# ZwwWayne/mmMOT

Measured on AMD Instinct MI355X. Metric: frame-pairs/sec (fusion+affinity fwd) at N_det=64; affinity L∞ vs CPU ref, higher is better.
Workload: dtype f16x3

## Files before the change

### include/mmmot_hip.h

```cpp
#ifndef MMMOT_HIP_H
#define MMMOT_HIP_H

#include <stddef.h>
#include <stdint.h>

#ifdef __cplusplus
extern "C" {
#endif

#define MMMOT_OK 0
#define MMMOT_EINVAL (-1)

#define MMMOT_ACT_NONE 0
#define MMMOT_ACT_RELU 1
#define MMMOT_ACT_SIGMOID 2

#define MMMOT_A_PLAIN 0
#define MMMOT_A_NORM_RELU 1
#define MMMOT_A_PAIR 2

#define MMMOT_PAIR_MULTIPLY 0
#define MMMOT_PAIR_MINUS_ABS 1
#define MMMOT_PAIR_MINUS 2

// ... 49 lines not shown
int mmmot_conv3x3_raw_hl16(const void* in, const void* wp, const float* bias, float* out, int L, int H, int W, int Cin,
                           int Cout, const float* oscale, void* stream);

typedef struct mmmot_gemm_args {
  const float* X; int ldx;
  const float* W;
  const float* bias;
  const float* dbias; const int* rowidx; int lddb;
  float* Y; int ldy;
  float* part;
  const float* sc; const float* sh; int ldsc;
  const float* FA; const float* FB; int ldf;
  const int* tile_row0; const int* tile_nrows; const int* tile_group;
  const int* grp_row0; const int* grp_M; const int* grp_aoff; const int* grp_boff;
  int T; int N; int K;
  int amode; int pairop; int act;
  int w_hl16; float oscale;
  const float* osc; const float* osh; int ldosc;
  float* colsum;
  int pair_uniform32;
} mmmot_gemm_args;
int mmmot_gemm_rows(const mmmot_gemm_args* a, void* stream);
int mmmot_set_gemm_rows_variant(int v);

typedef struct mmmot_gemm_ares_args {
  const float* X; int ldx;
  const float* sc; const float* sh; int ldsc;
  const void* W;
  const float* bias;
  const float* dbias; const int* tile_dbrow; int lddb;
  const int* tile_row0; const int* tile_nrows; const int* tile_group;
  float* part;
  const float* osc; const float* osh; int ldosc;
  float* colsum;
  int T; int N; int K;
  float oscale;
} mmmot_gemm_ares_args;
int mmmot_gemm_ares(const mmmot_gemm_ares_args* a, void* stream);
int mmmot_set_gemm_ares_variant(int v);

int mmmot_gram_rows(const float* X, int ldx, int K, const float* sc, const float* sh, int ldsc,
                    const int* tile_row0, const int* tile_nrows, const int* tile_group, int T,
                    double* Gout, double* Sout, void* stream);
int mmmot_set_gram128_variant(int v);
int mmmot_gn_finalize_gram(const double* Gp, const double* Sp, const int* grp_tile0, const int* grp_ntiles,
                           const int* grp_count, int G, int K, const float* W, const float* bias, int N,
// ... 9 lines not shown
                      const float* gamma, const float* beta, float eps,
                      float* sc, float* sh, void* stream);

int mmmot_segment_mean(const float* X, int ldx, int C,
                       const int* seg_start, const int* seg_count, const int* seg_stride,
                       const int* seg_group, const int* seg_div, int nseg,
                       const float* sc, const float* sh, int ldsc, int relu,
                       float* out, int ldo,
                       int hl16 ,
                       void* stream);

int mmmot_rowdot(const float* X, int ldx, int K, const float* w, float b,
                 const float* sc, const float* sh, int ldsc,
                 const int* tile_row0, const int* tile_nrows, const int* tile_group, int T,
                 int act, int use_thr, float thr,
                 float* out, const int* omap, void* stream);

int mmmot_row_layernorm(const float* X, int ldx, int C, const float* gamma, const float* beta,
                        float eps, int relu, float* Y, int ldy, int R, void* stream);

int mmmot_skippool_head(const float* P, int ldp, int C, int C4, const float* g0, const float* b0, const float* w1,
                        const float* c1, const float* g2, const float* b2, const float* w4, const float* c4,
                        const float* g5, const float* b5, float eps, float* out, int ldo, int R, void* stream);
int mmmot_pointnet_layer1(const float* X, int K, const float* W, const float* bias,
                          float* Y, float* part,
                          const int* tile_row0, const int* tile_nrows, int T, void* stream);

int mmmot_pn_mlp64(const float* X, int ldx, const float* sc, const float* sh, int ldsc, const void* W16,
                   float oscale, const float* bias, float* Y, int ldy, float* part, const int* tile_row0,
                   const int* tile_nrows, const int* tile_group, int T, int N, void* stream);

int mmmot_affine_act(const float* X, int ldx, int C, const float* sc, const float* sh, int ldsc,
                     const int* tile_row0, const int* tile_nrows, const int* tile_group, int T,
                     int act, float* Y, int ldy, void* stream);

int mmmot_fusion_combine(int mode, const float* cat, const float* Y0, int ld0,
                         const float* Y1, int ld1,
                         const float* sc0, const float* sh0, const float* sc1, const float* sh1, int ldsc,
                         const int* tile_row0, const int* tile_nrows, const int* tile_group, int T,
                         float* F, int Lt, int C, void* stream);

int mmmot_softmax_pairs(const float* logits, float* out,
                        const int* grp_row0, const int* grp_N, const int* grp_M, int G,
                        int max_nm ,
                        int mode, void* stream);

// ... 103 lines not shown
```

### mmmot_amd/_lib.py

```python
import ctypes
import os
import subprocess
import threading

_HERE = os.path.dirname(os.path.abspath(__file__))
CSRC = os.path.join(_HERE, 'csrc')
LIB_PATH = os.environ.get('MMMOT_LIB_PATH', os.path.join(_HERE, 'libmmmot_hip.so'))
SOURCES = ['conv3x3.hip', 'hl16_format.hip', 'conv3x3_hl16_patch.hip', 'gemm_rows.hip', 'gemm_wide.hip',
           'gemm_ares.hip', 'gemm_wres.hip', 'gemm_wreg.hip', 'pn_mlp64.hip', 'gram.hip', 'points_gather.hip', 'crop_resize.hip', 'small_kernels.hip', 'backward.hip', 'train.hip', 'train_vgg.hip', 'gemm_tn_f16.hip',
           'assign.hip', 'track_ids.hip']
HIPCC = os.environ.get('HIPCC', '/opt/rocm/bin/hipcc')
HIPFLAGS = ['--offload-arch=gfx950', '-O3', '-std=c++17', '-fPIC']

_lock = threading.Lock()
_lib = None

c_f = ctypes.c_void_p
c_i = ctypes.c_int


class GemmArgs(ctypes.Structure):
    _fields_ = [
        ('X', c_f), ('ldx', c_i),
        ('W', c_f),
# ... 23 lines not shown
        ('dbias', c_f), ('tile_dbrow', c_f), ('lddb', c_i),
        ('tile_row0', c_f), ('tile_nrows', c_f), ('tile_group', c_f),
        ('part', c_f),
        ('osc', c_f), ('osh', c_f), ('ldosc', c_i),
        ('colsum', c_f),
        ('T', c_i), ('N', c_i), ('K', c_i),
        ('oscale', ctypes.c_float),
    ]


class GemmTnArgs(ctypes.Structure):
    _fields_ = [
        ('dY', c_f), ('lddy', c_i),
        ('X', c_f), ('ldx', c_i),
        ('sc', c_f), ('sh', c_f), ('ldsc', c_i),
        ('FA', c_f), ('FB', c_f), ('ldf', c_i),
        ('tile_row0', c_f), ('tile_nrows', c_f), ('tile_group', c_f),
        ('grp_row0', c_f), ('grp_M', c_f), ('grp_aoff', c_f), ('grp_boff', c_f),
        ('T', c_i), ('N', c_i), ('K', c_i), ('amode', c_i), ('pairop', c_i), ('nsplit', c_i),
        ('dW', c_f), ('db', c_f),
    ]


SIGNATURES = {
    'mmmot_abi_version': [],
    'mmmot_device_info': [c_i, ctypes.POINTER(c_i), ctypes.c_char_p, c_i],
    'mmmot_conv3x3_bn_relu': [c_f, c_f, c_f, c_f, c_i, c_i, c_i, c_i, c_i, c_i, c_i, c_f],
    'mmmot_gemm_rows': [ctypes.POINTER(GemmArgs), c_f],
    'mmmot_set_gemm_rows_variant': [c_i],
    'mmmot_gemm_ares': [ctypes.POINTER(GemmAresArgs), c_f],
    'mmmot_set_gemm_ares_variant': [c_i],
    'mmmot_gram_rows': [c_f, c_i, c_i, c_f, c_f, c_i, c_f, c_f, c_f, c_i, c_f, c_f, c_f],
    'mmmot_set_gram128_variant': [c_i],
    'mmmot_gn_finalize_gram': [c_f, c_f, c_f, c_f, c_f, c_i, c_i, c_f, c_f, c_i, c_f, c_f, ctypes.c_float, c_f, c_f, c_f, c_f],
    'mmmot_gn_finalize_gram_dbias': [c_f, c_f, c_f, c_f, c_f, c_i, c_f, c_f, c_i, c_f, c_f, c_i, c_i, c_f, c_f, ctypes.c_float,
                                     c_f, c_f, c_f, c_f],
    'mmmot_gn_finalize': [c_f, c_f, c_f, c_f, c_f, c_i, c_i, c_i, c_i, c_f, c_f, ctypes.c_float, c_f, c_f, c_f],
    'mmmot_segment_mean': [c_f, c_i, c_i, c_f, c_f, c_f, c_f, c_f, c_i, c_f, c_f, c_i, c_i, c_f, c_i, c_i, c_f],
    'mmmot_conv3x3_bn_relu_hl16_patch': [c_f, c_f, c_f, c_f, c_i, c_i, c_i, c_i, c_i, c_i, c_f, c_f],
    'mmmot_conv1_fused_hl16': [c_f, c_f, c_f, ctypes.c_float, c_f, c_f, c_f, c_f, c_i, c_i, c_i, c_f],
    'mmmot_conv3x3_bn_relu_hq8': [c_f, c_f, c_f, c_f, c_i, c_i, c_i, c_i, c_i, c_i, c_f, c_f],
    'mmmot_conv1_fused_u8': [c_f, ctypes.c_float, ctypes.c_float, ctypes.c_float, ctypes.c_float, ctypes.c_float,
                             ctypes.c_float, c_f, c_f, ctypes.c_float, c_f, c_f, c_f, c_f, c_i, c_i, c_i, c_i, c_f],
    'mmmot_u8_normalize': [c_f, c_i, c_i, c_f, c_f, c_f],
    'mmmot_conv1_fused_hq8': [c_f, c_f, c_f, ctypes.c_float, c_f, c_f, c_f, c_f, c_i, c_i, c_i, c_f],
    'mmmot_conv3x3_first_hl16': [c_f, c_f, c_f, c_f, c_i, c_i, c_i, c_i, c_f],
    'mmmot_set_patch_grid_limit': [c_i],
    'mmmot_set_patch_min_block': [c_i],
    'mmmot_trunk_range_read': [ctypes.POINTER(ctypes.c_uint), c_i],
    'mmmot_trunk_range_bind': [c_f],
    'mmmot_hl16_pack': [c_f, c_f, ctypes.c_long, c_f],
    'mmmot_hl16_unpack': [c_f, c_f, ctypes.c_long, c_f],
    'mmmot_hl16_pack_pow2': [c_f, c_f, ctypes.c_long, c_f, c_i, c_f],
    'mmmot_pow2_oscale': [c_f, c_i, c_f, c_i, c_f, c_i, c_f],
    'mmmot_conv3x3_raw_hl16': [c_f, c_f, c_f, c_f, c_i, c_i, c_i, c_i, c_i, c_f, c_f],
    'mmmot_hq8_pack': [c_f, c_f, ctypes.c_long, c_f],
    'mmmot_hq8_unpack': [c_f, c_f, ctypes.c_long, c_f],
    'mmmot_rowdot': [c_f, c_i, c_i, c_f, ctypes.c_float, c_f, c_f, c_i, c_f, c_f, c_f, c_i, c_i, c_i,
                     ctypes.c_float, c_f, c_f, c_f],
    'mmmot_row_layernorm': [c_f, c_i, c_i, c_f, c_f, ctypes.c_float, c_i, c_f, c_i, c_i, c_f],
    'mmmot_skippool_head': [c_f, c_i, c_i, c_i, c_f, c_f, c_f, c_f, c_f, c_f, c_f, c_f, c_f, c_f, ctypes.c_float, c_f, c_i, c_i,
                            c_f],
    'mmmot_pointnet_layer1': [c_f, c_i, c_f, c_f, c_f, c_f, c_f, c_f, c_i, c_f],
    'mmmot_pn_mlp64': [c_f, c_i, c_f, c_f, c_i, c_f, ctypes.c_float, c_f, c_f, c_i, c_f, c_f, c_f, c_f, c_i, c_i, c_f],
    'mmmot_affine_act': [c_f, c_i, c_i, c_f, c_f, c_i, c_f, c_f, c_f, c_i, c_i, c_f, c_i, c_f],
    'mmmot_fusion_combine': [c_i, c_f, c_f, c_i, c_f, c_i, c_f, c_f, c_f, c_f, c_i, c_f, c_f, c_f, c_i, c_f,
                             c_i, c_i, c_f],
    'mmmot_softmax_pairs': [c_f, c_f, c_f, c_f, c_f, c_i, c_i, c_i, c_f],
    'mmmot_points_count': [c_f, c_i, c_i, c_f, c_i, c_i, c_f, c_f, c_f],
    'mmmot_points_scatter': [c_f, c_i, c_i, c_f, c_i, c_f, c_f, c_f, c_i, c_f],
    'mmmot_crop_resize_norm': [c_f, c_i, c_i, c_f, c_i, c_i, c_i, c_f, c_f, c_f, c_f, c_f],
    'mmmot_points_count_batched': [c_f, c_i, c_i, c_i, c_i, c_i, c_f, c_f, c_f, c_f, c_f, c_f, c_f, c_i, c_f, c_f, c_f],
    'mmmot_points_scatter_batched': [c_f, c_i, c_i, c_i, c_i, c_i, c_f, c_f, c_f, c_f, c_f, c_f, c_f, c_f, c_f, c_f, c_i, c_f],
    'mmmot_selftest_mfma': [c_f, c_f, c_f, c_i, c_f],
    'mmmot_gn_bwd_partial': [c_f, c_i, c_f, c_i, c_i, c_f, c_f, c_i, c_f, c_f, c_i, c_f, c_f, c_f, c_i, c_f, c_f],
    'mmmot_gn_bwd_finalize': [c_f, c_f, c_i, c_i, c_i, c_f, c_f, c_f],
    'mmmot_gn_bwd_apply': [c_f, c_i, c_f, c_i, c_i, c_f, c_f, c_i, c_f, c_f, c_i, c_f, c_f, c_f, c_f, c_i, c_f, c_i, c_f],
    'mmmot_gemm_tn': [ctypes.POINTER(GemmTnArgs), c_f],
    'mmmot_gemm_tn_f16': [ctypes.POINTER(GemmTnArgs), c_f, c_f],
    'mmmot_absmax': [c_f, c_i, ctypes.c_long, c_i, c_f, c_f],
    'mmmot_pair_bwd': [c_f, c_i, c_f, c_i, c_f, c_i, c_i, c_f, c_f, c_f, c_f, c_f, c_f, c_f, c_i, c_i, c_i, c_f],
    'mmmot_pair_expand_bwd': [c_f, c_i, c_f, c_i, c_i, c_f, c_f, c_f, c_i, c_f, c_f, c_f, c_f, c_f],
    'mmmot_rowdot_bwd': [c_f, c_i, c_i, c_f, ctypes.c_float, c_f, c_f, c_i, c_f, c_f, c_f, c_i, c_i, c_f, c_f, c_f, c_i,
                         c_f, c_i, c_f],
    'mmmot_softmax_pairs_bwd': [c_f, c_f, c_f, c_f, c_f, c_f, c_i, c_i, c_i, c_f],
# ... 86 lines not shown
```

### mmmot_amd/csrc/gemm_rows.hip

```cpp
#include "common.h"

#define G16_BK 64
#define G16_LDT 72

template <int BN, int AMODE, bool F16>
__global__ __launch_bounds__(MM_THREADS, 2) void gemm_rows_kernel(mmmot_gemm_args a, int ntn) {
  constexpr int WM = (BN == 128) ? 2 : 4;
  constexpr int WN = 4 / WM;
  constexpr int TM = MM_BM / (WM * 32);
  constexpr int TN = BN / (WN * 32);
  constexpr int BLD = BN / 32;
  constexpr int BK = F16 ? G16_BK : MM_BK;
  constexpr int KV = BK / 32;
  constexpr int SMEM_BYTES = F16 ? (MM_BM + BN) * G16_LDT * 2 * 2 : (MM_BM + BN) * MM_LDT * 4;
  constexpr bool STAGED_OUT = F16 && BN == 128;

  __shared__ __attribute__((aligned(16))) unsigned char smem_raw[SMEM_BYTES];
  float* smem = reinterpret_cast<float*>(smem_raw);
  float* As = smem;
  float* Bs = smem + MM_BM * MM_LDT;
  _Float16* hs = reinterpret_cast<_Float16*>(smem_raw);
  _Float16* As_hi = hs;
  _Float16* As_lo = hs + MM_BM * G16_LDT;
  _Float16* Bs_hi = hs + 2 * MM_BM * G16_LDT;
// ... 289 lines not shown
                acc[tm][tn][e];
      __syncthreads();
      constexpr int C4 = BN / 4;
      for (int w = tid; w < MM_BM * C4; w += MM_THREADS) {
        const int r = w / C4, c = (w - r * C4) * 4;
        if (r < nrows) {
          f32x4 v = *reinterpret_cast<const f32x4*>(&Cs[r * CLD + c]);
#pragma unroll
          for (int e = 0; e < 4; ++e) v[e] = mm_act(v[e], a.act);
          *reinterpret_cast<f32x4*>(&a.Y[(long)(row0 + r) * a.ldy + n0 + c]) = v;
        }
      }
    }
  }
}

template <int BN, int AMODE, bool F16>
static int launch_gemm(const mmmot_gemm_args* a, hipStream_t s) {
  const int ntn = a->N / BN;
  hipLaunchKernelGGL((gemm_rows_kernel<BN, AMODE, F16>), dim3(a->T * ntn), dim3(MM_THREADS), 0, s, *a, ntn);
  return mm_check(hipGetLastError());
}

template <bool F16>
static int dispatch_gemm(const mmmot_gemm_args* a, hipStream_t s) {
  const bool wide = (a->N % 128 == 0);
  switch (a->amode) {
    case MMMOT_A_PLAIN:
      return wide ? launch_gemm<128, MMMOT_A_PLAIN, F16>(a, s) : launch_gemm<64, MMMOT_A_PLAIN, F16>(a, s);
    case MMMOT_A_NORM_RELU:
      return wide ? launch_gemm<128, MMMOT_A_NORM_RELU, F16>(a, s) : launch_gemm<64, MMMOT_A_NORM_RELU, F16>(a, s);
    case MMMOT_A_PAIR:
      return wide ? launch_gemm<128, MMMOT_A_PAIR, F16>(a, s) : launch_gemm<64, MMMOT_A_PAIR, F16>(a, s);
  }
  return MMMOT_EINVAL;
}

int mmmot_gemm_wide_try(const mmmot_gemm_args* a, hipStream_t s, int* status);

extern "C" int mmmot_gemm_rows(const mmmot_gemm_args* a, void* stream) {
  hipStream_t s = (hipStream_t)stream;
  if (!a || !a->W || a->T <= 0 || !a->tile_row0 || !a->tile_nrows) return MMMOT_EINVAL;
  const int bk = a->w_hl16 ? G16_BK : MM_BK;
  if (a->K <= 0 || a->K % bk != 0 || a->N <= 0 || a->N % 64 != 0) return MMMOT_EINVAL;
  if (!mm_al16(a->W)) return MMMOT_EINVAL;
  if (a->amode == MMMOT_A_PAIR) {
    if (!a->FA || !a->FB || !a->grp_row0 || !a->grp_M || !a->grp_aoff || !a->grp_boff || !a->tile_group)
      return MMMOT_EINVAL;
    if (a->ldf % 4 != 0 || !mm_al16(a->FA) || !mm_al16(a->FB)) return MMMOT_EINVAL;
  } else {
    if (!a->X || a->ldx % 4 != 0 || !mm_al16(a->X)) return MMMOT_EINVAL;
    if (a->amode == MMMOT_A_NORM_RELU &&
        (!a->sc || !a->sh || a->ldsc % 4 != 0 || !mm_al16(a->sc) || !mm_al16(a->sh)))
      return MMMOT_EINVAL;
  }
  if (a->dbias && !a->rowidx) return MMMOT_EINVAL;
  if (a->colsum && (!a->osc || !a->osh)) return MMMOT_EINVAL;
// ... 32 lines not shown
```

### mmmot_amd/csrc/small_kernels.hip

```cpp
#include "common.h"

__global__ __launch_bounds__(256) void gn_finalize_kernel(
    const float* __restrict__ part, const int* __restrict__ grp_tile0, const int* __restrict__ grp_ntiles,
    const int* __restrict__ grp_count, const int* __restrict__ tile_nrows, int ldp, int C, int NG,
    const float* __restrict__ gamma, const float* __restrict__ beta, float eps, float* __restrict__ sc,
    float* __restrict__ sh) {
  __shared__ double red[2][4];
  const int g = blockIdx.x / NG, ng = blockIdx.x % NG;
  const int CG = C / NG, c0 = ng * CG;
  const int tile0 = grp_tile0[g], nt = grp_ntiles[g];
  const int tid = threadIdx.x, lane = tid & 63, wave = tid >> 6;
  const int rows = grp_count[g];
  const int dq = 256 / CG, dr = 256 % CG;
  const int ti0 = tid / CG, cc0 = tid % CG;
  constexpr int U = 16;
  double s1 = 0.0;
  {
    int ti = ti0, cc = cc0;
    while (ti < nt) {
      float v[U];
      int n = 0;
#pragma unroll
      for (int u = 0; u < U; ++u) {
        v[u] = 0.f;
// ... 467 lines not shown
        const bool up = (lane & o) != 0;
#pragma unroll
        for (int i = 0; i < o; ++i) {
          const float keep = up ? acc[i + o] : acc[i];
          const float send = up ? acc[i] : acc[i + o];
          acc[i] = keep + __shfl_xor(send, o);
        }
      }
      const int jb = lane / ROWS, rr = lane % ROWS;
      if (j0 + jb < N) out[rr][j0 + jb] = acc[0] + bias[j0 + jb];
    } else {
#pragma unroll
      for (int jb = 0; jb < JB; ++jb)
#pragma unroll
        for (int rr = 0; rr < ROWS; ++rr) {
          const float t = wave_sum(acc[jb * ROWS + rr]);
          if (lane == 0 && j0 + jb < N) out[rr][j0 + jb] = t + bias[j0 + jb];
        }
    }
  }
}

template <int ROWS>
__global__ __launch_bounds__(256) void skippool_head_kernel(
    const float* __restrict__ P, int ldp, int C, int C4, const float* __restrict__ g0, const float* __restrict__ b0,
    const float* __restrict__ w1, const float* __restrict__ c1, const float* __restrict__ g2,
    const float* __restrict__ b2, const float* __restrict__ w4, const float* __restrict__ c4,
    const float* __restrict__ g5, const float* __restrict__ b5, float eps, float* __restrict__ out, int ldo, int R) {
  constexpr int JB = ROWS == 8 ? 8 : SP_JB;
  constexpr int RW = ROWS < 4 ? 1 : ROWS / 4;
  __shared__ __attribute__((aligned(16))) float xs[ROWS][512];
  __shared__ __attribute__((aligned(16))) float hs[ROWS][512];
  __shared__ float h1[ROWS][128];
  const int lane = threadIdx.x & 63, wave = threadIdx.x >> 6;
  const int row0 = blockIdx.x * ROWS;
#pragma unroll
  for (int q = 0; q < RW; ++q) {
    const int lr = wave * RW + q;
    if (lr < ROWS) sp_layernorm_row(P + (long)(row0 + lr < R ? row0 + lr : 0) * ldp, C, g0, b0, eps, false, xs[lr], lane);
  }
  __syncthreads();
  sp_matvec<ROWS, JB>(w1, c1, C4, C, xs, h1, lane, wave);
  __syncthreads();
#pragma unroll
  for (int q = 0; q < RW; ++q) {
    const int lr = wave * RW + q;
    if (lr < ROWS) sp_layernorm_row(h1[lr], C4, g2, b2, eps, true, hs[lr], lane);
  }
  __syncthreads();
  sp_matvec<ROWS, JB>(w4, c4, 128, C4, hs, h1, lane, wave);
  __syncthreads();
#pragma unroll
  for (int q = 0; q < RW; ++q) {
    const int lr = wave * RW + q;
    if (lr < ROWS && row0 + lr < R) sp_layernorm_row(h1[lr], 128, g5, b5, eps, true, out + (long)(row0 + lr) * ldo, lane);
  }
}

extern "C" int mmmot_skippool_head(const float* P, int ldp, int C, int C4, const float* g0, const float* b0,
                                   const float* w1, const float* c1, const float* g2, const float* b2, const float* w4,
                                   const float* c4, const float* g5, const float* b5, float eps, float* out, int ldo,
                                   int R, void* stream) {
  if (!P || !g0 || !b0 || !w1 || !c1 || !g2 || !b2 || !w4 || !c4 || !g5 || !b5 || !out || R <= 0) return MMMOT_EINVAL;
  if (C <= 0 || C % 64 != 0 || C > 512 || C4 <= 0 || C4 % 64 != 0 || C4 > 128) return MMMOT_EINVAL;
  if (!mm_al16(w1) || !mm_al16(w4)) return MMMOT_EINVAL;
  if (R >= 256)
    hipLaunchKernelGGL(skippool_head_kernel<8>, dim3((R + 7) / 8), dim3(256), 0, (hipStream_t)stream, P, ldp,
                       C, C4, g0, b0, w1, c1, g2, b2, w4, c4, g5, b5, eps, out, ldo, R);
  else
    hipLaunchKernelGGL(skippool_head_kernel<SP_ROWS>, dim3((R + SP_ROWS - 1) / SP_ROWS), dim3(256), 0, (hipStream_t)stream,
                       P, ldp, C, C4, g0, b0, w1, c1, g2, b2, w4, c4, g5, b5, eps, out, ldo, R);
  return mm_check(hipGetLastError());
}

template <int K>
__global__ __launch_bounds__(256) void pointnet_layer1_kernel(
    const float* __restrict__ X, const float* __restrict__ W, const float* __restrict__ bias,
    float* __restrict__ Y, float* __restrict__ part, const int* __restrict__ tile_row0,
    const int* __restrict__ tile_nrows) {
  __shared__ float xs[MM_BM * K];
  __shared__ float red[4][2][64];
  const int t = blockIdx.x;
  const int row0 = tile_row0[t], nrows = tile_nrows[t];
  const int tid = threadIdx.x;
  for (int idx = tid; idx < nrows * K; idx += 256) xs[idx] = X[(long)row0 * K + idx];
  __syncthreads();
  const int c = tid & 63, rq = tid >> 6;
  float w[K];
#pragma unroll
  for (int k = 0; k < K; ++k) w[k] = W[c * K + k];
  const float bv = bias[c];
  auto val = [&](int r) {
    float y = bv;
#pragma unroll
// ... 212 lines not shown
```

### mmmot_amd/engine.py

```python
import contextlib
import itertools
import os
import threading

import numpy as np
import torch

from .ops import (ACT_NONE, ACT_RELU, ACT_SIGMOID, A_NORM_RELU, A_PAIR, A_PLAIN, FUSION_MODES, PAIR_OPS,
                  SOFTMAX_MODES)
from .range_guard import RangeGuard
from .tape import norm_layer

POOL_INPUT = {'f32': 0, 'hl16': 1, 'hq8': 2}
EPS = 1e-5
_SERIALS = itertools.count(1)


def check_crop_side(S):
    if S < 32 or S % 2 != 0:
        raise ValueError('crop side %d is not supported: the HIP VGG trunk needs an even side >= 32; resize the crops '
                         '(mmmot_amd.crops.crop_resize_normalize)' % S)


def check_crop_layout(dets):
    if dets.dtype == torch.uint8:
        if dets.dim() != 4 or dets.shape[3] != 3 or dets.shape[1] != dets.shape[2]:
            raise ValueError('uint8 crops must be [L,S,S,3] (HWC, the output of mmmot_amd.crops.crop_resize_u8), got %s'
                             % (tuple(dets.shape),))
        S = int(dets.shape[1])
    else:
        S = int(dets.shape[-1])
    check_crop_side(S)
# ... 9 lines not shown
        if trunk not in ('f16x3', 'f16q8', 'f32'):
            raise ValueError("trunk must be 'f16x3' (fp16 matrix cores, 3-term split), 'f16q8' (fp16 main term + "
                             "fp8 correction terms, include/mmmot_hip.h hq8) or 'f32' (exact fp32 MFMA)")
        self.trunk = trunk
        self.serial = next(_SERIALS)
        self.trunk_requested = trunk
        self.guard = RangeGuard(self)
        self.range_events = []
        self.last_out_of_range_forward = None
        self.out_of_range_window = None
        self._busy = threading.Lock()
        self._last_stream = None
        self._image_token = None
        self._pre_image = None
        ql = os.environ.get('MMMOT_Q8_LAYERS', '4,5,6,7,8,9,10,11,12')
        self.q8_layers = None if ql == 'all' else set(int(v) for v in ql.split(',') if v)
        self.pn_fused = os.environ.get('MMMOT_PN_FUSED', '1') != '0'
        self.pn_gram = os.environ.get('MMMOT_PN_GRAM', '1') != '0'
        self.pn_mlp64 = os.environ.get('MMMOT_PN_MLP64', '1') != '0'
        self.two_streams = os.environ.get('MMMOT_TWO_STREAMS', '0') == '1'
        self.pn_beside_trunk = os.environ.get('MMMOT_PN_BESIDE_TRUNK', '1') != '0'
        self._side = {}
        self.sp_fused = os.environ.get('MMMOT_SP_FUSED', '1') != '0'
        self.fuse_conv1 = os.environ.get('MMMOT_FUSE_CONV1', '1') != '0'
        self.q8_min_crop = int(os.environ.get('MMMOT_Q8_MIN_CROP', '64'))
        self.mlp = 'f32' if trunk == 'f32' else 'f16x3'
        if affinity_op not in PAIR_OPS:
            raise ValueError('unknown affinity_op %r' % (affinity_op,))
        if softmax_mode not in SOFTMAX_MODES and softmax_mode != 'none':
            softmax_mode = 'none'
        self.end_mode = end_mode
        self.P = packed
        self.ops = ops
        self.fusion = fusion
        self.affinity_op = affinity_op
        self.softmax_mode = softmax_mode
        self.neg_threshold = float(neg_threshold)
        self.score_arch = score_arch
        self.ws = {}
        self.dev = None
        self.keep = None
        self._tape = None
        self.conv_events = None

    def buf(self, name, *shape, device=None, dtype=torch.float32):
        if self._tape is not None:
# ... 63 lines not shown
        if self.keep is not None:
            self.keep[key] = t.detach().clone()
        if self._tape is not None:
            self._tape[key] = t

    def appearance(self, plan, crops, cat):
        ops, Lt, S = self.ops, plan.Lt, plan.S
        check_crop_side(S)
        if Lt * S * S * 16 >= 2 ** 31 - 64:
            raise ValueError('%d crops of %dx%d in one launch sequence exceed the 32-bit piece offsets of the trunk kernels '
                             '(L*S*S*16 < 2^31): split the batch' % (Lt, S, S))
        x, H, W = crops, S, S
        u8 = crops.dtype == torch.uint8
        q8 = self.q8_in_force(S)
        f16 = self.trunk in ('f16x3', 'f16q8')
        vgg = self.P['vgg']
        fuse1 = (f16 and self.fuse_conv1 and len(vgg) > 1 and vgg[0]['cout'] == 64 and
                 vgg[1]['cin'] == 64 and vgg[1]['cout'] == 64 and vgg[1]['pool'] and not vgg[0]['last'] and
                 not vgg[0]['pool'])
        if u8 and not fuse1:
            x = self.buf('vgg_crops32', Lt, 3, S, S)
            ops.u8_normalize(crops, self._mean_std(crops.device), x, Lt, S)
            u8 = False
        fmt = 'raw'
        for li, cv in enumerate(vgg):
            if fuse1 and li == 0:
                continue
            lq8 = q8 and (self.q8_layers is None or li in self.q8_layers)
            want = 'hq8' if lq8 else 'hl16'
            if f16 and fmt in ('hl16', 'hq8') and fmt != want:
                n = Lt * H * W * cv['cin']
                tmp = self.buf('vgg_recode32', n)
                (ops.hq8_unpack if fmt == 'hq8' else ops.hl16_unpack)(x, tmp)
                x = self.buf('vgg_recode', n)
                (ops.hq8_pack if want == 'hq8' else ops.hl16_pack)(tmp, x)
                fmt = want
            Ho, Wo = (H // 2, W // 2) if cv['pool'] else (H, W)
            out = self.buf('vgg%d' % (li & 1), Lt * Ho * Wo, cv['cout'])
            if self.conv_events is not None:
                e0, e1 = torch.cuda.Event(enable_timing=True), torch.cuda.Event(enable_timing=True)
                e0.record()
            if fuse1 and li == 1:
                c0 = vgg[0]
                if u8:
                    from .crops import MEAN, STD
                    ops.conv1_fused_u8(x, MEAN, STD, c0['wp16'], c0['bias'], c0['oscale'], cv['wpq8'] if lq8 else cv['wp16'],
# ... 10 lines not shown
                if nq8:
                    tmp = self.buf('vgg_first32', Lt * H * W, cv['cout'])
                    ops.conv3x3(x, cv['wp'], cv['bias'], tmp, Lt, H, W, cv['cin'], cv['cout'], True, cv['pool'])
                    ops.hq8_pack(tmp, out)
                else:
                    ops.conv3x3_first_hl16(x, cv['wp'], cv['bias'], out, Lt, H, W, cv['cout'])
                fmt = 'hq8' if nq8 else 'hl16'
            elif lq8:
                ops.conv3x3_hq8(x, cv['wpq8'], cv['bias'], out, Lt, H, W, cv['cin'], cv['cout'], cv['pool'], cv['oscale'])
                fmt = 'hq8'
            elif not f16:
                ops.conv3x3(x, cv['wp'], cv['bias'], out, Lt, H, W, cv['cin'], cv['cout'], li == 0, cv['pool'])
                fmt = 'f32'
            else:
                ops.conv3x3_hl16_patch(x, cv['wp16'], cv['bias'], out, Lt, H, W, cv['cin'], cv['cout'], cv['pool'],
                                       cv['oscale'])
                fmt = 'hl16'
            if self.conv_events is not None:
                e1.record()
                self.conv_events.append((li, Lt * H * W, cv['cin'], cv['cout'], e0, e1))
            x, H, W = out, Ho, Wo
            if cv['last']:
                self._stash('vgg_stage%d' % cv['stage'], x)
                self._skippool(plan, cv['stage'], x, H * W, cv['cout'], cat, fmt)

    def _mean_std(self, dev):
        key = ('mean_std', str(dev))
        if key not in self.ws:
            from .crops import MEAN, STD
            self.ws[key] = torch.tensor(list(MEAN) + list(STD), dtype=torch.float32, device=dev)
        return self.ws[key]

    def q8_in_force(self, S):
        return self.trunk == 'f16q8' and S >= self.q8_min_crop

    def trunk_elements(self, plan):
        n, H = 0, plan.S
        for cv in self.P['vgg']:
            if cv['pool']:
                H //= 2
            n += plan.Lt * H * H * cv['cout']
        return n

    def _skippool(self, plan, s, x, hw, C, cat, fmt='f32'):
        hl16 = POOL_INPUT[fmt]
        ops, Lt, hd, T = self.ops, plan.Lt, self.P['skippool'][s], plan.det_tiles
        pooled = self.buf('sp_pool', Lt, C)
        first, second, npart = plan.crop_segments(hw)
        if second is None:
            ops.segment_mean(x, C, first, pooled, use_group=False, hl16=hl16)
        else:
            partial = self.buf('sp_partial', npart, C)
            ops.segment_mean(x, C, first, partial, use_group=False, hl16=hl16)
            ops.segment_mean(partial, C, second, pooled, use_group=False)
        if self.sp_fused and hasattr(ops, 'skippool_head'):
            ops.skippool_head(pooled, C, hd, EPS, cat[:, 128 * s:128 * (s + 1)], Lt)
            return
        ln0 = self.buf('sp_ln0', Lt, C)
        ops.row_layernorm(pooled, C, hd['g0'], hd['b0'], EPS, False, ln0, Lt)
        C4 = hd['w1'].shape[0]
        h1 = self.buf('sp_h1', Lt, C4)
        self._gemm(hd, 'w1', T, C4, C, X=ln0, bias=hd['c1'], Y=h1)
        ln1 = self.buf('sp_ln1', Lt, C4)
        ops.row_layernorm(h1, C4, hd['g2'], hd['b2'], EPS, True, ln1, Lt)
        h2 = self.buf('sp_h2', Lt, 128)
        self._gemm(hd, 'w4', T, 128, C4, X=ln1, bias=hd['c4'], Y=h2)
        ops.row_layernorm(h2, 128, hd['g5'], hd['b5'], EPS, True, cat[:, 128 * s:128 * (s + 1)], Lt)

    def pointnet(self, plan, points, cat):
        ops, pn, T, D, Pn, Lt = self.ops, self.P['pointnet'], plan.pt_tiles, plan.det_tiles, plan.P, plan.Lt
        y1 = self.buf('pn_y1', Pn, 64)
        part = self._part(T, 64)
        ops.pointnet_layer1(points, pn['w1'], pn['b1'], y1, part, T)
        sc1, sh1 = self._finalize('pn1', part, T, 64, 64, pn['g1'], pn['be1'])
        x, sc, sh = y1, sc1, sh1
        for i, (N, K) in zip((2, 3, 4), ((64, 64), (64, 64), (128, 64))):
            y = self.buf('pn_y%d' % i, Pn, N)
# ... 306 lines not shown
```

### mmmot_amd/ops.py

```python
import contextlib
import ctypes
import os
import threading

import torch

from . import _lib

ACT_NONE, ACT_RELU, ACT_SIGMOID = 0, 1, 2
A_PLAIN, A_NORM_RELU, A_PAIR = 0, 1, 2
PAIR_OPS = {'multiply': 0, 'minus_abs': 1, 'minus': 2}
SOFTMAX_MODES = {'single': 1, 'dual': 2, 'dual_add': 3, 'dual_max': 4}
FUSION_MODES = {'A': 0, 'B': 1, 'C': 2}
LOSS_KINDS = {'bce': 0, 'l2': 1, 'l1': 2}


def _ptr(t, dtype=torch.float32):
    if t is None:
        return None
    if not t.is_cuda:
        raise RuntimeError('mmmot_amd HIP ops need device tensors (got %s); there is no CPU fallback' % t.device)
    if t.dtype != dtype:
        raise TypeError('expected %s, got %s' % (dtype, t.dtype))
    return t.data_ptr()
# ... 3 lines not shown
    return _ptr(t, torch.int32)


def _ld(t):
    if t is None:
        return 0
    if t.dim() == 1:
        return t.shape[0]
    if t.dim() != 2 or (t.shape[1] > 1 and t.stride(1) != 1):
        raise ValueError('expected a 2-D view with unit inner stride, got shape %s stride %s' % (
            tuple(t.shape), tuple(t.stride())))
    return t.stride(0)


class HipOps:
    name = 'hip'

    def __init__(self):
        self.lib = _lib.load()
        self._osvecs = {}
        self._scr = {}
        self.tn_f16 = os.environ.get('MMMOT_GEMM_TN', 'f16x3') != 'f32'
        self._tls = threading.local()

    @property
    def _pinned_stream(self):
        return getattr(self._tls, 'stream', None)

    @_pinned_stream.setter
    def _pinned_stream(self, v):
        self._tls.stream = v

    def _scratch(self, name, n, device):
        key = (name, n, str(device))
        t = self._scr.get(key)
        if t is None:
            t = self._scr[key] = torch.empty(n, dtype=torch.float32, device=device)
        return t

    def _osv(self, oscale, Cout, like):
        if torch.is_tensor(oscale):
            if oscale.numel() != Cout:
                raise ValueError('oscale must hold one scale per output channel')
            return oscale
        key = (float(oscale), Cout, like.device)
        v = self._osvecs.get(key)
# ... 188 lines not shown
                                         _iptr(getattr(segs, 'div', None)), segs.n,
                                         _ptr(sc), _ptr(sh), _ld(sc), int(bool(relu)) | (2 if take_max else 0), _ptr(out), _ld(out),
                                         int(hl16), self._stream())
        _lib.check(st, 'mmmot_segment_mean')

    def rowdot(self, X, K, w, b, tiles, out, sc=None, sh=None, act=ACT_NONE, use_thr=False, thr=0.0, omap=None):
        st = self.lib.mmmot_rowdot(_ptr(X), _ld(X), K, _ptr(w), float(b), _ptr(sc), _ptr(sh), _ld(sc),
                                   _iptr(tiles.row0), _iptr(tiles.nrows), _iptr(tiles.group), tiles.T, act,
                                   int(use_thr), float(thr), _ptr(out), _iptr(omap), self._stream())
        _lib.check(st, 'mmmot_rowdot')

    def row_layernorm(self, X, C, gamma, beta, eps, relu, Y, R):
        st = self.lib.mmmot_row_layernorm(_ptr(X), _ld(X), C, _ptr(gamma), _ptr(beta), float(eps), int(relu),
                                          _ptr(Y), _ld(Y), R, self._stream())
        _lib.check(st, 'mmmot_row_layernorm')

    def skippool_head(self, P, C, hd, eps, out, R):
        C4 = int(hd['w1'].shape[0])
        st = self.lib.mmmot_skippool_head(_ptr(P), _ld(P), C, C4, _ptr(hd['g0']), _ptr(hd['b0']), _ptr(hd['w1']),
                                          _ptr(hd['c1']), _ptr(hd['g2']), _ptr(hd['b2']), _ptr(hd['w4']), _ptr(hd['c4']),
                                          _ptr(hd['g5']), _ptr(hd['b5']), float(eps), _ptr(out), _ld(out), R, self._stream())
        _lib.check(st, 'mmmot_skippool_head')

    def pointnet_layer1(self, X, W, bias, Y, part, tiles):
        st = self.lib.mmmot_pointnet_layer1(_ptr(X), int(W.shape[1]), _ptr(W), _ptr(bias), _ptr(Y), _ptr(part),
                                            _iptr(tiles.row0), _iptr(tiles.nrows), tiles.T, self._stream())
        _lib.check(st, 'mmmot_pointnet_layer1')

    def affine_act(self, X, C, sc, sh, tiles, act, Y):
        st = self.lib.mmmot_affine_act(_ptr(X), _ld(X), C, _ptr(sc), _ptr(sh), _ld(sc), _iptr(tiles.row0),
                                       _iptr(tiles.nrows), _iptr(tiles.group), tiles.T, act, _ptr(Y), _ld(Y),
                                       self._stream())
        _lib.check(st, 'mmmot_affine_act')

    def fusion_combine(self, mode, cat, Y0, Y1, sc0, sh0, sc1, sh1, tiles, F, Lt, C):
        st = self.lib.mmmot_fusion_combine(mode, _ptr(cat), _ptr(Y0), _ld(Y0), _ptr(Y1), _ld(Y1), _ptr(sc0),
                                           _ptr(sh0), _ptr(sc1), _ptr(sh1), _ld(sc0), _iptr(tiles.row0),
                                           _iptr(tiles.nrows), _iptr(tiles.group), tiles.T, _ptr(F), Lt, C,
                                           self._stream())
        _lib.check(st, 'mmmot_fusion_combine')

    def softmax_pairs(self, logits, out, row0, gN, gM, G, max_nm, mode):
        st = self.lib.mmmot_softmax_pairs(_ptr(logits), _ptr(out), _iptr(row0), _iptr(gN), _iptr(gM), G,
                                          max_nm, mode, self._stream())
        _lib.check(st, 'mmmot_softmax_pairs')

# ... 145 lines not shown
```

### mmmot_amd/profiler.py

```python
import time

import torch

PEAK_F16X3_TFLOPS = 2500.0 / 3.0
PEAK_F32_TFLOPS = 157.3
PEAK_HBM_TBS = 8.0


def _rows(t):
    return int(getattr(t, 'R', 0))


def _seg_rows(segs):
    return int(segs.h_count.sum())


def _conv(name):
    def cost(a, k):
        inp, wp, bias, out, L, H, W, Cin, Cout = a[:9]
        pool = a[10] if name == 'conv3x3' else a[9]
        Ho, Wo = (H // 2, W // 2) if pool else (H, W)
        fl = 2.0 * L * H * W * 9 * Cin * Cout
        by = 4.0 * (L * H * W * Cin + L * Ho * Wo * Cout + 9 * Cin * Cout)
        return ('trunk conv %d->%d @%dx%d%s' % (Cin, Cout, H, W, ' +pool' if pool else ''), fl, by)
# ... 66 lines not shown
    return ('PointNet layer %d->64 (points in)' % Kin, 2.0 * R * Kin * 64, 4.0 * R * (Kin + 64))


COSTS = {
    'conv3x3': _conv('conv3x3'),
    'conv3x3_hl16_patch': _conv('hl16'),
    'conv3x3_hq8': _conv('hq8'),
    'conv1_fused_hl16': _conv1_fused,
    'conv1_fused_hq8': _conv1_fused,
    'conv1_fused_u8': _conv1_fused,
    'conv3x3_first_hl16': lambda a, k: ('trunk conv1_1 3->%d (fp32 MFMA)' % a[7], 2.0 * a[4] * a[5] * a[6] * 27 * a[7],
                                        4.0 * a[4] * a[5] * a[6] * (3 + a[7])),
    'gemm': _gemm,
    'gemm_ares': _gemm_ares,
    'pn_mlp64': _pn_mlp64,
    'gram_rows': _gram,
    'gn_finalize_gram': _latency('GroupNorm scale/shift from the Gram matrix'),
    'gn_finalize_gram_dbias': _latency('GroupNorm scale/shift from the Gram matrix'),
    'gn_finalize': _latency('GroupNorm scale/shift from tile partials'),
    'segment_mean': _segment_mean,
    'rowdot': _rowdot,
    'row_layernorm': _latency('row LayerNorm'),
    'skippool_head': _latency('SkipPool head (LN, 1x1, LN, 1x1, LN)'),
    'pointnet_layer1': _layer1,
    'affine_act': _latency('affine + activation rows'),
    'fusion_combine': _latency('fusion combine'),
    'softmax_pairs': _latency('pair softmax'),
    'u8_normalize': _latency('8-bit crops -> fp32'),
    'hq8_pack': _latency('hq8 / hl16 re-encode'), 'hq8_unpack': _latency('hq8 / hl16 re-encode'),
    'hl16_pack': _latency('hq8 / hl16 re-encode'), 'hl16_unpack': _latency('hq8 / hl16 re-encode'),
}


class LaunchProfiler:

    def __init__(self, ops, f32=False):
        self.ops = ops
        self.cuda = torch.cuda.is_available()
        self.peak_tf = PEAK_F32_TFLOPS if f32 else PEAK_F16X3_TFLOPS
        self.records = []
        self._saved = {}

    def _wrap(self, name, fn, cost):
        def wrapped(*a, **k):
            try:
                label, fl, by = cost(a, k)
# ... 76 lines not shown
```

Before: 296.9.

## Batch SkipPool heads into one launch and narrow GEMM column tiles for occupancy

All per-stage SkipPool head launches are collected and issued as a single grid, with blockIdx.y selecting the stage and each stage's pooled buffer kept separately, which removes several small kernel launches. Separately, gemm_rows now shrinks its column tile from 128 or 64 down to 32 when the tile count would not cover the CU count, adding more blocks for small-N_det workloads. The trade-off is smaller tiles with less reuse per block, plus extra pooled buffers.

New measurement: 297.8 (median of 5 runs). About the same (+0.3%).

```diff
diff --git a/include/mmmot_hip.h b/include/mmmot_hip.h
--- a/include/mmmot_hip.h
+++ b/include/mmmot_hip.h
@@ -95,6 +95,7 @@
 } mmmot_gemm_args;
 int mmmot_gemm_rows(const mmmot_gemm_args* a, void* stream);
 int mmmot_set_gemm_rows_variant(int v);
+int mmmot_set_gemm_rows_narrow(int v);
 
 typedef struct mmmot_gemm_ares_args {
   const float* X; int ldx;
@@ -150,6 +151,16 @@
 int mmmot_skippool_head(const float* P, int ldp, int C, int C4, const float* g0, const float* b0, const float* w1,
                         const float* c1, const float* g2, const float* b2, const float* w4, const float* c4,
                         const float* g5, const float* b5, float eps, float* out, int ldo, int R, void* stream);
+
+#define MMMOT_SKIPPOOL_MAX_STAGES 4
+typedef struct {
+  const float* P;
+  int ldp, C, C4;
+  const float *g0, *b0, *w1, *c1, *g2, *b2, *w4, *c4, *g5, *b5;
+  float* out;
+  int ldo;
+} mmmot_skippool_stage;
+int mmmot_skippool_heads(const mmmot_skippool_stage* stages, int nstages, float eps, int R, void* stream);
 int mmmot_pointnet_layer1(const float* X, int K, const float* W, const float* bias,
                           float* Y, float* part,
                           const int* tile_row0, const int* tile_nrows, int T, void* stream);
diff --git a/mmmot_amd/_lib.py b/mmmot_amd/_lib.py
--- a/mmmot_amd/_lib.py
+++ b/mmmot_amd/_lib.py
@@ -69,12 +69,20 @@
     ]
 
 
+class SkipPoolStage(ctypes.Structure):
+    _fields_ = [('P', c_f), ('ldp', c_i), ('C', c_i), ('C4', c_i)] + \
+        [(n, c_f) for n in ('g0', 'b0', 'w1', 'c1', 'g2', 'b2', 'w4', 'c4', 'g5', 'b5')] + [('out', c_f), ('ldo', c_i)]
+
+
+SKIPPOOL_MAX_STAGES = 4
+
 SIGNATURES = {
     'mmmot_abi_version': [],
     'mmmot_device_info': [c_i, ctypes.POINTER(c_i), ctypes.c_char_p, c_i],
     'mmmot_conv3x3_bn_relu': [c_f, c_f, c_f, c_f, c_i, c_i, c_i, c_i, c_i, c_i, c_i, c_f],
     'mmmot_gemm_rows': [ctypes.POINTER(GemmArgs), c_f],
     'mmmot_set_gemm_rows_variant': [c_i],
+    'mmmot_set_gemm_rows_narrow': [c_i],
     'mmmot_gemm_ares': [ctypes.POINTER(GemmAresArgs), c_f],
     'mmmot_set_gemm_ares_variant': [c_i],
     'mmmot_gram_rows': [c_f, c_i, c_i, c_f, c_f, c_i, c_f, c_f, c_f, c_i, c_f, c_f, c_f],
@@ -108,6 +116,7 @@
     'mmmot_row_layernorm': [c_f, c_i, c_i, c_f, c_f, ctypes.c_float, c_i, c_f, c_i, c_i, c_f],
     'mmmot_skippool_head': [c_f, c_i, c_i, c_i, c_f, c_f, c_f, c_f, c_f, c_f, c_f, c_f, c_f, c_f, ctypes.c_float, c_f, c_i, c_i,
                             c_f],
+    'mmmot_skippool_heads': [ctypes.POINTER(SkipPoolStage), c_i, ctypes.c_float, c_i, c_f],
     'mmmot_pointnet_layer1': [c_f, c_i, c_f, c_f, c_f, c_f, c_f, c_f, c_i, c_f],
     'mmmot_pn_mlp64': [c_f, c_i, c_f, c_f, c_i, c_f, ctypes.c_float, c_f, c_f, c_i, c_f, c_f, c_f, c_f, c_i, c_i, c_f],
     'mmmot_affine_act': [c_f, c_i, c_i, c_f, c_f, c_i, c_f, c_f, c_f, c_i, c_i, c_f, c_i, c_f],
diff --git a/mmmot_amd/csrc/gemm_rows.hip b/mmmot_amd/csrc/gemm_rows.hip
--- a/mmmot_amd/csrc/gemm_rows.hip
+++ b/mmmot_amd/csrc/gemm_rows.hip
@@ -1,4 +1,6 @@
 #include "common.h"
+#include <atomic>
+#include <cstdlib>
 
 #define G16_BK 64
 #define G16_LDT 72
@@ -335,17 +337,42 @@
   return mm_check(hipGetLastError());
 }
 
+static std::atomic<int> g_rows_narrow{-1};
+extern "C" int mmmot_set_gemm_rows_narrow(int v) {
+  if (v < 0) return MMMOT_EINVAL;
+  g_rows_narrow.store(v);
+  return MMMOT_OK;
+}
+
+static int rows_col_tile(const mmmot_gemm_args* a) {
+  int bn = (a->N % 128 == 0) ? 128 : 64;
+  int narrow = g_rows_narrow.load();
+  if (narrow < 0) {
+    const char* e = getenv("MMMOT_GEMM_NARROW");
+    narrow = e ? atoi(e) : 1;
+    if (narrow < 0) narrow = 1;
+    g_rows_narrow.store(narrow);
+  }
+  if (narrow == 0 || a->colsum) return bn;
+  const long want = narrow == 1 ? mm_num_cu() : narrow;
+  while (bn > 32 && (long)a->T * (a->N / bn) < want) bn >>= 1;
+  return bn;
+}
+
 template <bool F16>
 static int dispatch_gemm(const mmmot_gemm_args* a, hipStream_t s) {
-  const bool wide = (a->N % 128 == 0);
+  const int bn = rows_col_tile(a);
+#define MM_ROWS_CASE(MODE)                                        \
+  case MODE:                                                      \
+    return bn == 128  ? launch_gemm<128, MODE, F16>(a, s)         \
+           : bn == 64 ? launch_gemm<64, MODE, F16>(a, s)          \
+                      : launch_gemm<32, MODE, F16>(a, s);
   switch (a->amode) {
-    case MMMOT_A_PLAIN:
-      return wide ? launch_gemm<128, MMMOT_A_PLAIN, F16>(a, s) : launch_gemm<64, MMMOT_A_PLAIN, F16>(a, s);
-    case MMMOT_A_NORM_RELU:
-      return wide ? launch_gemm<128, MMMOT_A_NORM_RELU, F16>(a, s) : launch_gemm<64, MMMOT_A_NORM_RELU, F16>(a, s);
-    case MMMOT_A_PAIR:
-      return wide ? launch_gemm<128, MMMOT_A_PAIR, F16>(a, s) : launch_gemm<64, MMMOT_A_PAIR, F16>(a, s);
-  }
+    MM_ROWS_CASE(MMMOT_A_PLAIN)
+    MM_ROWS_CASE(MMMOT_A_NORM_RELU)
+    MM_ROWS_CASE(MMMOT_A_PAIR)
+  }
+#undef MM_ROWS_CASE
   return MMMOT_EINVAL;
 }
 
diff --git a/mmmot_amd/csrc/small_kernels.hip b/mmmot_amd/csrc/small_kernels.hip
--- a/mmmot_amd/csrc/small_kernels.hip
+++ b/mmmot_amd/csrc/small_kernels.hip
@@ -513,18 +513,18 @@
 }
 
 template <int ROWS>
-__global__ __launch_bounds__(256) void skippool_head_kernel(
+__device__ __forceinline__ void sp_head_rows(
     const float* __restrict__ P, int ldp, int C, int C4, const float* __restrict__ g0, const float* __restrict__ b0,
     const float* __restrict__ w1, const float* __restrict__ c1, const float* __restrict__ g2,
     const float* __restrict__ b2, const float* __restrict__ w4, const float* __restrict__ c4,
-    const float* __restrict__ g5, const float* __restrict__ b5, float eps, float* __restrict__ out, int ldo, int R) {
+    const float* __restrict__ g5, const float* __restrict__ b5, float eps, float* __restrict__ out, int ldo, int R,
+    int row0) {
   constexpr int JB = ROWS == 8 ? 8 : SP_JB;
   constexpr int RW = ROWS < 4 ? 1 : ROWS / 4;
   __shared__ __attribute__((aligned(16))) float xs[ROWS][512];
   __shared__ __attribute__((aligned(16))) float hs[ROWS][512];
   __shared__ float h1[ROWS][128];
   const int lane = threadIdx.x & 63, wave = threadIdx.x >> 6;
-  const int row0 = blockIdx.x * ROWS;
 #pragma unroll
   for (int q = 0; q < RW; ++q) {
     const int lr = wave * RW + q;
@@ -546,6 +546,26 @@
     const int lr = wave * RW + q;
     if (lr < ROWS && row0 + lr < R) sp_layernorm_row(h1[lr], 128, g5, b5, eps, true, out + (long)(row0 + lr) * ldo, lane);
   }
+}
+
+template <int ROWS>
+__global__ __launch_bounds__(256) void skippool_head_kernel(
+    const float* __restrict__ P, int ldp, int C, int C4, const float* __restrict__ g0, const float* __restrict__ b0,
+    const float* __restrict__ w1, const float* __restrict__ c1, const float* __restrict__ g2,
+    const float* __restrict__ b2, const float* __restrict__ w4, const float* __restrict__ c4,
+    const float* __restrict__ g5, const float* __restrict__ b5, float eps, float* __restrict__ out, int ldo, int R) {
+  sp_head_rows<ROWS>(P, ldp, C, C4, g0, b0, w1, c1, g2, b2, w4, c4, g5, b5, eps, out, ldo, R, blockIdx.x * ROWS);
+}
+
+struct sp_heads_table {
+  mmmot_skippool_stage st[MMMOT_SKIPPOOL_MAX_STAGES];
+};
+
+template <int ROWS>
+__global__ __launch_bounds__(256) void skippool_heads_kernel(sp_heads_table tb, float eps, int R) {
+  const mmmot_skippool_stage& h = tb.st[blockIdx.y];
+  sp_head_rows<ROWS>(h.P, h.ldp, h.C, h.C4, h.g0, h.b0, h.w1, h.c1, h.g2, h.b2, h.w4, h.c4, h.g5, h.b5, eps, h.out, h.ldo, R,
+                     blockIdx.x * ROWS);
 }
 
 extern "C" int mmmot_skippool_head(const float* P, int ldp, int C, int C4, const float* g0, const float* b0,
@@ -561,6 +581,26 @@
   else
     hipLaunchKernelGGL(skippool_head_kernel<SP_ROWS>, dim3((R + SP_ROWS - 1) / SP_ROWS), dim3(256), 0, (hipStream_t)stream,
                        P, ldp, C, C4, g0, b0, w1, c1, g2, b2, w4, c4, g5, b5, eps, out, ldo, R);
+  return mm_check(hipGetLastError());
+}
+
+extern "C" int mmmot_skippool_heads(const mmmot_skippool_stage* stages, int nstages, float eps, int R, void* stream) {
+  if (!stages || nstages <= 0 || nstages > MMMOT_SKIPPOOL_MAX_STAGES || R <= 0) return MMMOT_EINVAL;
+  sp_heads_table tb;
+  for (int i = 0; i < nstages; ++i) {
+    const mmmot_skippool_stage& h = stages[i];
+    if (!h.P || !h.g0 || !h.b0 || !h.w1 || !h.c1 || !h.g2 || !h.b2 || !h.w4 || !h.c4 || !h.g5 || !h.b5 || !h.out)
+      return MMMOT_EINVAL;
+    if (h.C <= 0 || h.C % 64 != 0 || h.C > 512 || h.C4 <= 0 || h.C4 % 64 != 0 || h.C4 > 128) return MMMOT_EINVAL;
+    if (!mm_al16(h.w1) || !mm_al16(h.w4)) return MMMOT_EINVAL;
+    tb.st[i] = h;
+  }
+  for (int i = nstages; i < MMMOT_SKIPPOOL_MAX_STAGES; ++i) tb.st[i] = stages[0];
+  if (R >= 256)
+    hipLaunchKernelGGL(skippool_heads_kernel<8>, dim3((R + 7) / 8, nstages), dim3(256), 0, (hipStream_t)stream, tb, eps, R);
+  else
+    hipLaunchKernelGGL(skippool_heads_kernel<SP_ROWS>, dim3((R + SP_ROWS - 1) / SP_ROWS, nstages), dim3(256), 0,
+                       (hipStream_t)stream, tb, eps, R);
   return mm_check(hipGetLastError());
 }
 
diff --git a/mmmot_amd/engine.py b/mmmot_amd/engine.py
--- a/mmmot_amd/engine.py
+++ b/mmmot_amd/engine.py
@@ -8,6 +8,7 @@
 
 from .ops import (ACT_NONE, ACT_RELU, ACT_SIGMOID, A_NORM_RELU, A_PAIR, A_PLAIN, FUSION_MODES, PAIR_OPS,
                   SOFTMAX_MODES)
+from ._lib import SKIPPOOL_MAX_STAGES
 from .range_guard import RangeGuard
 from .tape import norm_layer
 
@@ -63,6 +64,7 @@
         self.pn_beside_trunk = os.environ.get('MMMOT_PN_BESIDE_TRUNK', '1') != '0'
         self._side = {}
         self.sp_fused = os.environ.get('MMMOT_SP_FUSED', '1') != '0'
+        self.sp_heads = os.environ.get('MMMOT_SP_HEADS', '1') != '0'
         self.fuse_conv1 = os.environ.get('MMMOT_FUSE_CONV1', '1') != '0'
         self.q8_min_crop = int(os.environ.get('MMMOT_Q8_MIN_CROP', '64'))
         self.mlp = 'f32' if trunk == 'f32' else 'f16x3'
@@ -172,6 +174,8 @@
             x = self.buf('vgg_crops32', Lt, 3, S, S)
             ops.u8_normalize(crops, self._mean_std(crops.device), x, Lt, S)
             u8 = False
+        heads = [] if (self.sp_fused and self.sp_heads and getattr(ops, 'skippool_heads', None) is not None and
+                       len(self.P['skippool']) <= SKIPPOOL_MAX_STAGES) else None
         fmt = 'raw'
         for li, cv in enumerate(vgg):
             if fuse1 and li == 0:
@@ -228,7 +232,9 @@
             x, H, W = out, Ho, Wo
             if cv['last']:
                 self._stash('vgg_stage%d' % cv['stage'], x)
-                self._skippool(plan, cv['stage'], x, H * W, cv['cout'], cat, fmt)
+                self._skippool(plan, cv['stage'], x, H * W, cv['cout'], cat, fmt, heads)
+        if heads:
+            ops.skippool_heads(heads, EPS, Lt)
 
     def _mean_std(self, dev):
         key = ('mean_std', str(dev))
@@ -248,10 +254,10 @@
             n += plan.Lt * H * H * cv['cout']
         return n
 
-    def _skippool(self, plan, s, x, hw, C, cat, fmt='f32'):
+    def _skippool(self, plan, s, x, hw, C, cat, fmt='f32', heads=None):
         hl16 = POOL_INPUT[fmt]
         ops, Lt, hd, T = self.ops, plan.Lt, self.P['skippool'][s], plan.det_tiles
-        pooled = self.buf('sp_pool', Lt, C)
+        pooled = self.buf('sp_pool' if heads is None else 'sp_pool%d' % s, Lt, C)
         first, second, npart = plan.crop_segments(hw)
         if second is None:
             ops.segment_mean(x, C, first, pooled, use_group=False, hl16=hl16)
@@ -259,6 +265,9 @@
             partial = self.buf('sp_partial', npart, C)
             ops.segment_mean(x, C, first, partial, use_group=False, hl16=hl16)
             ops.segment_mean(partial, C, second, pooled, use_group=False)
+        if heads is not None:
+            heads.append((pooled, C, hd, cat[:, 128 * s:128 * (s + 1)]))
+            return
         if self.sp_fused and hasattr(ops, 'skippool_head'):
             ops.skippool_head(pooled, C, hd, EPS, cat[:, 128 * s:128 * (s + 1)], Lt)
             return
diff --git a/mmmot_amd/ops.py b/mmmot_amd/ops.py
--- a/mmmot_amd/ops.py
+++ b/mmmot_amd/ops.py
@@ -49,6 +49,8 @@
         self._scr = {}
         self.tn_f16 = os.environ.get('MMMOT_GEMM_TN', 'f16x3') != 'f32'
         self._tls = threading.local()
+        if not hasattr(self.lib, 'mmmot_skippool_heads'):
+            self.skippool_heads = None
 
     @property
     def _pinned_stream(self):
@@ -283,6 +285,15 @@
                                           _ptr(hd['g5']), _ptr(hd['b5']), float(eps), _ptr(out), _ld(out), R, self._stream())
         _lib.check(st, 'mmmot_skippool_head')
 
+    def skippool_heads(self, stages, eps, R):
+        tb = (_lib.SkipPoolStage * len(stages))()
+        for st, (P, C, hd, out) in zip(tb, stages):
+            st.P, st.ldp, st.C, st.C4 = _ptr(P), _ld(P), C, int(hd['w1'].shape[0])
+            for k in ('g0', 'b0', 'w1', 'c1', 'g2', 'b2', 'w4', 'c4', 'g5', 'b5'):
+                setattr(st, k, _ptr(hd[k]))
+            st.out, st.ldo = _ptr(out), _ld(out)
+        _lib.check(self.lib.mmmot_skippool_heads(tb, len(stages), float(eps), R, self._stream()), 'mmmot_skippool_heads')
+
     def pointnet_layer1(self, X, W, bias, Y, part, tiles):
         st = self.lib.mmmot_pointnet_layer1(_ptr(X), int(W.shape[1]), _ptr(W), _ptr(bias), _ptr(Y), _ptr(part),
                                             _iptr(tiles.row0), _iptr(tiles.nrows), tiles.T, self._stream())
diff --git a/mmmot_amd/profiler.py b/mmmot_amd/profiler.py
--- a/mmmot_amd/profiler.py
+++ b/mmmot_amd/profiler.py
@@ -112,6 +112,7 @@
     'rowdot': _rowdot,
     'row_layernorm': _latency('row LayerNorm'),
     'skippool_head': _latency('SkipPool head (LN, 1x1, LN, 1x1, LN)'),
+    'skippool_heads': _latency('SkipPool head (LN, 1x1, LN, 1x1, LN)'),
     'pointnet_layer1': _layer1,
     'affine_act': _latency('affine + activation rows'),
     'fusion_combine': _latency('fusion combine'),
```
